# PeterChg/koordinator

Measured on AMD Instinct MI355X. Metric: pod×node Filter+Score evals/sec (LoadAwareScheduling + NodeResourcesFit, matrix mode), higher is better.
Workload: dtype int64

## Files before the change

koordinator_amd/csrc/kg_engine.hip:

```cpp
#include <dlfcn.h>
#include <hip/hip_runtime.h>
#include <rccl/rccl.h>
#include <stdarg.h>
#include <stdio.h>
#include <string.h>

#include <algorithm>
#include <map>
#include <unordered_map>
#include <utility>
#include <string>
#include <type_traits>
#include <vector>

#include "kg_comm.h"
#include "kg_common.h"
#include "kg_host.h"

#define KG_POD_CHUNK 64
#define KG_RESOLVE_THREADS 512
#define KG_RESOLVE_LA_T0 448
#define KG_CLS_ITEM_MAX 512
#define KG_MAX_CHUNK KG_PLACE_CHUNK_MAX
#define KG_MAX_TILES 4096
// ... 1386 lines not shown
    }
    if (live && best && KG_IN2(88, p, a.n_pods, tile, a.tiles_total)) atomicMax(&partials[(int64_t)p * a.tiles_total + tile], best);
}

template <bool COMBINE>
__global__ __launch_bounds__(256) __attribute__((amdgpu_waves_per_eu(KG_NUMA2_WPE))) void k_eval_numa2(kg_consts c, kg_planes pl, HotArgs a,
                                                    const kg_pod_dev *__restrict__ pods,
                                                    const kg_node_row *__restrict__ rows,
                                                    unsigned long long *__restrict__ mask,
                                                    uint16_t *__restrict__ scores, uint8_t *__restrict__ numa_scores,
                                                    uint32_t *__restrict__ partials, const int32_t *__restrict__ perm,
                                                    BatchMasks bm, int32_t *queue, int32_t n_items, int32_t seg) {
    const int tid = threadIdx.x, lane = tid & 63;
    const int wave = __builtin_amdgcn_readfirstlane(tid >> 6);
    __shared__ kg_zone_tab_data ztab[256 / 64];
    __shared__ __attribute__((aligned(16))) uint4 lrow_s[256 / 64][KG_NUMA2_PREFETCH ? 2 : 1][64];
    static_assert(sizeof(kg_node_row) % 16 == 0 && sizeof(kg_node_row) <= 64 * 16, "rows are staged as 16-byte words");
    const int n_pb = (a.n_pods + 63) / 64;
    for (int it = 0;; it++) {
        int64_t tile, base;
        int npw, pb;
        if (queue == nullptr) {
            if (it > 0) break;
            tile = (int64_t)a.tile_begin + blockIdx.x;
            pb = blockIdx.y;
            npw = KG_NUMA2_NODES / (int)gridDim.z;
            base = tile * KG_TILE + wave * KG_NUMA2_NODES + (int64_t)blockIdx.z * npw;
        } else {
            int item = 0;
            if (lane == 0) item = atomicAdd(queue, 1);
            item = __builtin_amdgcn_readfirstlane(item);
            if (item >= n_items) break;
            pb = item % n_pb;
            const int run = item / n_pb;
            tile = (int64_t)a.tile_begin + run / (KG_TILE / seg);
            base = (int64_t)a.tile_begin * KG_TILE + (int64_t)run * seg;
            npw = seg;
        }
        const int slot = pb * 64 + lane;
        const bool live = slot < a.n_pods;
        const int p = live && perm ? perm[slot] : slot;
        const kg_pod_dev pd = pods[live ? p : 0];
        numa2_run<COMBINE>(c, pl, a, pd, p, live, tile, base, npw, rows, mask, scores, numa_scores, partials, bm, ztab[wave],
                  &lrow_s[wave][0][0]);
    }
}

__device__ __forceinline__ unsigned long long decode_partial(uint32_t k, int tile) {
    if (k == 0) return 0ull;
    const uint32_t node = (uint32_t)tile * KG_TILE + (KG_TILE - 1) - (k & (KG_TILE - 1));
    return ((unsigned long long)(k >> KG_TILE_SHIFT) << 32) | (0xFFFFFFFFull - node);
}

__global__ void k_top1(const uint32_t *__restrict__ partials, int32_t tiles, int32_t n_pods,
                       unsigned long long *__restrict__ out) {
    const int wave = (blockIdx.x * blockDim.x + threadIdx.x) >> 6;
    const int lane = threadIdx.x & 63;
    if (wave >= n_pods) return;
    unsigned long long best = 0;
    for (int t = lane; t < tiles; t += 64) {
        unsigned long long k = KG_IN2(89, wave, n_pods, t, tiles) ? decode_partial(partials[(int64_t)wave * tiles + t], t) : 0ull;
        best = best > k ? best : k;
    }
    best = wave_max_u64(best);
    if (lane == 0 && KG_IN(90, wave, n_pods)) out[wave] = best;
}

template <bool NUMA>
__device__ unsigned long long pair_key(const kg_consts &c, const kg_planes &pl, const kg_pod_dev &p, int64_t node,
                                       int64_t n_nodes, int64_t now_ns) {
    if (node < 0 || node >= n_nodes) return 0ull;
    NodeRegs n;
    BatchMasks bm{0xFFu, 0xFFu};
    load_node(c, pl, node, true, bm, now_ns, n);
    uint32_t fit, la, numa = 0;
    if (!eval_pair(c, pl, p, n, node, now_ns, fit, la)) return 0ull;
    if (NUMA && (c.plugins & KG_PLUGIN_NUMA)) {
        const uint64_t ns = kg_numa_eval_any(c, pl.rows[node], p);
        if (!(ns >> 32)) return 0ull;
        numa = (uint32_t)ns;
    }
    return ((unsigned long long)(total_of(c, fit, la, numa) + 1u) << 32) | (0xFFFFFFFFull - (unsigned long long)node);
}

#define KG_NUMA_CHUNK_PODS 16
#define KG_CHUNK_WPE 3
template <bool BZ>
__global__ __launch_bounds__(256) __attribute__((amdgpu_waves_per_eu(KG_CHUNK_WPE))) void k_eval_numa_chunk(kg_consts c, kg_planes pl, HotArgs a,
                                                         const kg_pod_dev *__restrict__ pods, int32_t shard_tiles,
                                                         uint32_t *__restrict__ partials) {
    __shared__ __attribute__((aligned(16))) kg_pod_dev lp;
    __shared__ __attribute__((aligned(16))) uint32_t kbuf[KG_TILE];
    const int tid = threadIdx.x, lane = tid & 63;
    const int n = a.n_pods;
    const int b = blockIdx.x, xcd = b % KG_XCDS, r = b / KG_XCDS;
    const int tile_rel = (r / n) * KG_XCDS + xcd, p = r % n;
    if (tile_rel >= shard_tiles) return;
    constexpr int POD_DW = (int)(sizeof(kg_pod_dev) / 4);
    for (int k = tid; k < POD_DW; k += 256)
        reinterpret_cast<uint32_t *>(&lp)[k] = reinterpret_cast<const uint32_t *>(pods + p)[k];
    __syncthreads();
    const int tile = a.tile_begin + tile_rel;
    const BatchMasks bm{0xFFu, 0xFFu};
#pragma unroll 1
    for (int v = 0; v < KG_TILE / 256; v++) {
        const int local = v * 256 + tid;
        const int64_t node = (int64_t)tile * KG_TILE + local;
        const bool in_range = node < a.node_end;
        NodeRegs nr;
        load_node(c, pl, node, in_range, bm, a.now_ns, nr);
        uint32_t key = 0;
        uint32_t fit, la;
        if (in_range && eval_pair(c, pl, lp, nr, node, a.now_ns, fit, la)) {
// ... 1122 lines not shown
    kg_pod_dev *pods = nullptr;
    void *hot = nullptr;
    int32_t nslot = 2;
    int32_t slot_res[8] = {0, 1, -1, -1, -1, -1, -1, -1};
    int32_t n_pods = 0, pods_cap = 0;
    size_t hot_bytes = 0;
    int32_t *numa_perm = nullptr;
    bool numa_perm_on = false;
    bool eq_on = false;
    int32_t eq_n = 0;
    kg_pod_dev *eq_pods = nullptr;
    void *eq_hot = nullptr;
    bool reps_in = false;
    int32_t *eq_perm = nullptr;
    bool eq_perm_on = false;
    int32_t *eq_of = nullptr;
    void *eq_mem = nullptr;
    size_t eq_mem_bytes = 0;
    void *ncache_mem = nullptr;
    size_t ncache_bytes = 0;
    uint8_t *ncache = nullptr;
    int64_t ncache_stride = 0;
    bool ncache_live = false;
    BatchMasks bm{0, 0};
    uint32_t forms = 0;
    int64_t numa_resident_wgs = 0;
    int64_t numa_resident_wgs_c = 0;
    int32_t *numa_queue = nullptr;
    int32_t numa_chunk_pods = KG_NUMA_CHUNK_PODS;
    bool la_prod = false;
    bool pow2 = true;
    bool cls_ok = false;
    bool cls_dirty = true;
    int64_t cls_width = -1, cls_tiles = -1;
    std::vector<kg_cls_desc> cls_desc;
    std::vector<std::vector<int32_t>> cls_members;
    std::vector<std::vector<int32_t>> cls_ux;
    std::vector<std::vector<int32_t>> cls_reps;
    std::vector<kg_pod_row> pod_rows_h;
    void *cls_mem = nullptr;
    size_t cls_mem_bytes = 0;
    int32_t cls_nwork = 0;
    int32_t cls_nids = 0;
    int32_t cls_kind_work[12][2] = {};
    size_t cls_work_off = 0, cls_rows_off = 0, cls_ids_off = 0;
    int32_t *xslow_list = nullptr;
    int32_t *xslow_count = nullptr;
    double *hot_lax = nullptr;
    bool lax_ok = false;
    int32_t lax_n = 0, lax_x[KG_LAX] = {};
    int32_t *slow_list = nullptr;
    int32_t *slow_count = nullptr;
    bool slow_valid = false;
    void *scratch = nullptr;
    size_t scratch_bytes = 0;
    uint64_t generation = 0;
    bool stale = false;
    std::vector<uint8_t> node_bind_facts;
    int64_t n_numa_policy_nodes = 0, n_node_bind_nodes = 0, n_no_detail_nodes = 0;
    bool batch_bind = false;
    struct CpuTable {
        int32_t max_ref = 1, strategy = KG_STRATEGY_LEAST_ALLOCATED;
        std::vector<kg_cpu_info> cpus;
    };
    std::unordered_map<int32_t, CpuTable> cpu_tab;
    std::vector<uint8_t> pod_may_bind;
    bool profiling = false;
    int64_t cls_target_blocks = 2048, cls_dup_target_blocks = 4096;
    hipStream_t stream2 = nullptr;
    hipEvent_t ev_fork = nullptr, ev_join = nullptr;
    hipEvent_t ev_res[3] = {};
    void *rsv_mem = nullptr;
    kg_reservation *rsv = nullptr;
    std::vector<int32_t> rsv_perm;
    int32_t n_rsv = 0;
    int32_t *rfirst = nullptr, *rnode = nullptr;
    int32_t n_rn = 0;
    unsigned long long *rsv_e = nullptr;
    int64_t *rsv_o = nullptr;
    kg_rsv_ment *rsv_m = nullptr;
    int32_t *rsv_mn = nullptr;
    unsigned long long *rsv_g = nullptr;
    kg_quota *quota = nullptr;
    int32_t n_quota = 0;
    int32_t max_pod_quota = -1;
    uint8_t *gate = nullptr;
    kg_counters ctr{};
    int64_t ev_acc = 0;
    ncclComm_t comm = nullptr;
    kg_shm_comm *shm = nullptr;
    uint32_t *shm_stage = nullptr;
    uint32_t *comm_word = nullptr;
    unsigned long long *cyc_words = nullptr;
    kg_cycle_out *cyc_out = nullptr;
    int32_t comm_rank = 0, comm_world = 0;
    hipStream_t eval_stream = nullptr;
    static constexpr int kEvalEvents = 4;
    hipEvent_t ev_eval[kEvalEvents] = {};
    const void *ev_eval_buf[kEvalEvents] = {};
    int32_t ev_eval_next = 0;
    static constexpr int kRing = 256;
    hipEvent_t ev0[kRing] = {}, ev1[kRing] = {};
    int64_t ev_count = 0;
    std::string err;
};

// ... 428 lines not shown
    e->cls_width = width;
    e->cls_tiles = shard_tiles;
    e->cls_dirty = false;
    return KG_OK;
}

template <bool MOST, bool FIT_ON, bool LA_ON, bool W1, int KIND, int FORM>
void launch_cls_kind(kg_engine *e, dim3 grid, const HotArgs &a_in, const kg_cls_desc *descs, const kg_cls_work *work,
                     const char *rows, const int32_t *ids, uint64_t *mask, uint16_t *scores, uint32_t *partials,
                     hipStream_t stream) {
    constexpr bool LAU = FORM == 1;
    const int32_t first = e->cls_kind_work[3 * KIND + FORM][0], count = e->cls_kind_work[3 * KIND + FORM][1];
    if (count == 0) return;
#ifdef KG_BOUNDS_CHECK
    HotArgs a = a_in;
    a.cls_ndesc = (int32_t)e->cls_desc.size();
    a.cls_nwork = count;
    a.cls_nids = e->cls_nids;
#else
    const HotArgs &a = a_in;
#endif
    if constexpr (LAU && !LA_ON) return;
    else if constexpr (FORM == 2) {
        const dim3 g1((unsigned)((count + KG_XCDS - 1) / KG_XCDS * KG_XCDS));
        if (mask)
            hipLaunchKernelGGL((k_eval3_dup<MOST, FIT_ON, LA_ON, true, W1, KIND>), g1, dim3(KG_TILE / 2), 0, stream,
                               e->consts, e->pl, a, descs, work + first, count, rows, ids, mask, scores, partials);
        else
            hipLaunchKernelGGL((k_eval3_dup<MOST, FIT_ON, LA_ON, false, W1, KIND>), g1, dim3(KG_TILE / 2), 0, stream,
                               e->consts, e->pl, a, descs, work + first, count, rows, ids, mask, scores, partials);
    } else {
        grid.y = (unsigned)count;
        if (mask)
            hipLaunchKernelGGL((k_eval3<MOST, FIT_ON, LA_ON, true, W1, KIND, LAU>), grid, dim3(KG_TILE / 2), 0, stream,
                               e->consts, e->pl, a, descs, work + first, rows, ids, mask, scores, partials);
        else
            hipLaunchKernelGGL((k_eval3<MOST, FIT_ON, LA_ON, false, W1, KIND, LAU>), grid, dim3(KG_TILE / 2), 0, stream,
                               e->consts, e->pl, a, descs, work + first, rows, ids, mask, scores, partials);
    }
}

template <bool MOST, bool FIT_ON, bool LA_ON, bool W1>
void launch_cls4(kg_engine *e, dim3 grid, const HotArgs &a, uint64_t *mask, uint16_t *scores, uint32_t *partials) {
    const char *m = (const char *)e->cls_mem;
    const kg_cls_desc *descs = (const kg_cls_desc *)m;
    const kg_cls_work *work = (const kg_cls_work *)(m + e->cls_work_off);
    const char *rows = m + e->cls_rows_off;
    const int32_t *ids = (const int32_t *)(m + e->cls_ids_off);
    if (!e->stream2) {
        (void)hipStreamCreateWithFlags(&e->stream2, hipStreamNonBlocking);
        (void)hipEventCreateWithFlags(&e->ev_fork, hipEventDisableTiming);
        (void)hipEventCreateWithFlags(&e->ev_join, hipEventDisableTiming);
    }
    (void)hipEventRecord(e->ev_fork, e->stream);
    (void)hipStreamWaitEvent(e->stream2, e->ev_fork, 0);
    hipStream_t s2 = e->stream2;
#define KG_LAUNCH_KIND(K)                                                                                              \
    launch_cls_kind<MOST, FIT_ON, LA_ON, W1, K, 2>(e, grid, a, descs, work, rows, ids, mask, scores, partials, e->stream); \
    launch_cls_kind<MOST, FIT_ON, LA_ON, W1, K, 1>(e, grid, a, descs, work, rows, ids, mask, scores, partials, e->stream); \
    launch_cls_kind<MOST, FIT_ON, LA_ON, W1, K, 0>(e, grid, a, descs, work, rows, ids, mask, scores, partials, s2)
    KG_LAUNCH_KIND(0);
    KG_LAUNCH_KIND(1);
    KG_LAUNCH_KIND(2);
    KG_LAUNCH_KIND(3);
#undef KG_LAUNCH_KIND
    (void)hipEventRecord(e->ev_join, s2);
    (void)hipStreamWaitEvent(e->stream, e->ev_join, 0);
}

template <bool MOST, bool FIT_ON, bool LA_ON>
void launch_cls3(kg_engine *e, dim3 grid, const HotArgs &a, uint64_t *mask, uint16_t *scores, uint32_t *partials) {
    bool unit = e->consts.weight_fit == 1 && e->consts.weight_la == 1;
    if (LA_ON) unit = unit && e->consts.la_w[0] == 1 && e->consts.la_w[1] == 1;
    for (const kg_cls_desc &d : e->cls_desc)
        for (int f = 0; f < 4; f++) unit = unit && d.fit_w[f] <= 1u && d.uni_w[f] <= 1u;
    if (unit) launch_cls4<MOST, FIT_ON, LA_ON, true>(e, grid, a, mask, scores, partials);
    else launch_cls4<MOST, FIT_ON, LA_ON, false>(e, grid, a, mask, scores, partials);
}

void launch_cls(kg_engine *e, dim3 grid, const HotArgs &a, uint64_t *mask, uint16_t *scores, uint32_t *partials) {
    const bool most = e->consts.fit_most != 0;
    const bool fit = (e->consts.plugins & KG_PLUGIN_FIT) != 0, la = (e->consts.plugins & KG_PLUGIN_LOADAWARE) != 0;
    if (!fit) launch_cls3<false, false, true>(e, grid, a, mask, scores, partials);
    else if (most && la) launch_cls3<true, true, true>(e, grid, a, mask, scores, partials);
    else if (most) launch_cls3<true, true, false>(e, grid, a, mask, scores, partials);
    else if (la) launch_cls3<false, true, true>(e, grid, a, mask, scores, partials);
    else launch_cls3<false, true, false>(e, grid, a, mask, scores, partials);
}

kg_status slow_refresh(kg_engine *e) {
    if (e->slow_valid) return KG_OK;
    HIP_TRY(e, hipMemsetAsync(e->slow_count, 0, sizeof(int32_t), e->stream));
    if (e->n_nodes > 0)
        hipLaunchKernelGGL(k_slow_list, dim3((unsigned)((e->n_nodes + 255) / 256)), dim3(256), 0, e->stream, e->pl.dflags,
                           (int64_t)0, e->n_nodes, e->slow_list, e->slow_count);
    HIP_TRY(e, hipGetLastError());
    e->slow_valid = true;
    return KG_OK;
}

kg_status launch_eval_plain(kg_engine *e, int64_t now_ns, int32_t pod_begin, int32_t n, uint64_t *mask, uint16_t *scores,
                            uint32_t *partials, bool use_cls, bool topk, HotArgs a, int64_t shard_tiles, bool prof = true) {
    if (e->consts.la_extra && !topk && e->lax_ok) {
        a.lax_n = e->lax_n;
        for (int k = 0; k < KG_LAX; k++) {
            a.lax_x[k] = k < e->lax_n ? e->lax_x[k] : 0;
            a.lax_w[k] = k < e->lax_n ? (uint32_t)e->consts.la_wx[e->lax_x[k]] : 0u;
        }
        a.lax_est = e->hot_lax + (int64_t)pod_begin * KG_LAX;
        if (prof && e->profiling) HIP_TRY(e, prof_begin(e));
        dim3 grid((unsigned)shard_tiles, (unsigned)((n + a.pods_per_block - 1) / a.pods_per_block));
        const bool prod = e->la_prod;
#define KG_LAX_LAUNCH(S_)                                                                                               \
        do {                                                                                                            \
            const kg_pod_hot_t<S_> *hp = reinterpret_cast<const kg_pod_hot_t<S_> *>(e->hot) + pod_begin;                \
            if (mask && prod)                                                                                          \
                hipLaunchKernelGGL((k_eval2<S_, false, true, true, false, true>), grid, dim3(KG_BLOCK), 0, e->stream,  \
                                   e->consts, e->pl, a, hp, mask, scores, partials);                                   \
            else if (mask)                                                                                             \
                hipLaunchKernelGGL((k_eval2<S_, false, false, true, false, true>), grid, dim3(KG_BLOCK), 0, e->stream, \
                                   e->consts, e->pl, a, hp, mask, scores, partials);                                   \
            else if (prod)                                                                                             \
                hipLaunchKernelGGL((k_eval2<S_, false, true, false, false, true>), grid, dim3(KG_BLOCK), 0, e->stream, \
                                   e->consts, e->pl, a, hp, mask, scores, partials);                                   \
            else                                                                                                       \
                hipLaunchKernelGGL((k_eval2<S_, false, false, false, false, true>), grid, dim3(KG_BLOCK), 0, e->stream,\
                                   e->consts, e->pl, a, hp, mask, scores, partials);                                   \
        } while (0)
        if (e->nslot == 2) KG_LAX_LAUNCH(2);
        else if (e->nslot == 4) KG_LAX_LAUNCH(4);
        else KG_LAX_LAUNCH(8);
#undef KG_LAX_LAUNCH
        HIP_TRY(e, hipGetLastError());
        if (prof && e->profiling) HIP_TRY(e, prof_end(e));
        HIP_TRY(e, hipMemsetAsync(e->xslow_count, 0, sizeof(int32_t), e->stream));
        if (e->n_nodes > 0)
            hipLaunchKernelGGL(k_slow_list, dim3((unsigned)((e->n_nodes + 255) / 256)), dim3(256), 0, e->stream, e->pl.dflags,
                               (int64_t)0, e->n_nodes, e->xslow_list, e->xslow_count, (uint32_t)KGD_XSLOW);
        hipLaunchKernelGGL(k_fix_slow, dim3((unsigned)((n + 255) / 256)), dim3(256), 0, e->stream, e->consts, e->pl,
                           e->pods + pod_begin, n, e->xslow_list, e->xslow_count, e->shard_begin, e->shard_end,
                           a.mask_words, a.score_stride, a.tiles_total, now_ns, (unsigned long long *)mask, scores,
                           partials);
        HIP_TRY(e, hipGetLastError());
        return KG_OK;
    }
    if (e->consts.la_extra && !topk) {
        if (prof && e->profiling) HIP_TRY(e, prof_begin(e));
        const int64_t width = e->shard_end - e->shard_begin;
        dim3 grid((unsigned)((width + 255) / 256), (unsigned)(n < 65535 ? n : 65535));
        hipLaunchKernelGGL(k_eval_exact, grid, dim3(256), 0, e->stream, e->consts, e->pl, e->pods + pod_begin, n,
                           e->shard_begin, e->shard_end, a.mask_words, a.score_stride, a.tiles_total, now_ns,
                           (unsigned long long *)mask, scores, partials);
        HIP_TRY(e, hipGetLastError());
        if (prof && e->profiling) HIP_TRY(e, prof_end(e));
        return KG_OK;
    }
    use_cls = use_cls && e->cls_ok && !e->reps_in && pod_begin == 0 && n == e->n_pods;
    if (use_cls) {
        kg_status st = cls_layout(e, e->shard_end - e->shard_begin, shard_tiles);
        if (st) return st;
    }
    dim3 grid((unsigned)shard_tiles, use_cls ? (unsigned)e->cls_nwork : (unsigned)((n + a.pods_per_block - 1) / a.pods_per_block));
    if (prof && e->profiling) HIP_TRY(e, prof_begin(e));
    if (use_cls) launch_cls(e, grid, a, mask, scores, partials);
    else if (e->nslot == 2) launch_hot<2>(e, grid, a, pod_begin, mask, scores, partials, topk);
    else if (e->nslot == 4) launch_hot<4>(e, grid, a, pod_begin, mask, scores, partials, topk);
    else launch_hot<8>(e, grid, a, pod_begin, mask, scores, partials, topk);
    HIP_TRY(e, hipGetLastError());
    if (prof && e->profiling) HIP_TRY(e, prof_end(e));
    kg_status st = slow_refresh(e);
    if (st) return st;
    if (!topk) {
        hipLaunchKernelGGL(k_fix_slow, dim3((unsigned)((n + 255) / 256)), dim3(256), 0, e->stream, e->consts, e->pl,
                           e->pods + pod_begin, n, e->slow_list, e->slow_count, e->shard_begin, e->shard_end,
                           a.mask_words, a.score_stride, a.tiles_total, now_ns, (unsigned long long *)mask, scores,
                           partials);
        HIP_TRY(e, hipGetLastError());
    }
    return KG_OK;
}

kg_status launch_eval(kg_engine *e, int64_t now_ns, int32_t pod_begin, int32_t n, uint64_t *mask, uint16_t *scores,
                      uint32_t *partials, bool use_cls = false, uint8_t *numa_scores = nullptr, bool topk = false) {
    if (n <= 0) return KG_OK;
    if ((mask == nullptr) != (scores == nullptr)) return set_err(e, KG_ERR_INVALID_ARG, "mask and scores go together");
    const int64_t shard_tiles = (e->shard_end - e->shard_begin + KG_TILE - 1) / KG_TILE;
    if (shard_tiles <= 0) return KG_OK;
    HotArgs a;
    a.n_pods = n;
    a.pods_per_block = pods_per_block_for(n, shard_tiles);
    a.tile_begin = (int32_t)(e->shard_begin / KG_TILE);
    a.tiles_total = (int32_t)tiles_total(e);
    a.node_end = e->shard_end;
    a.col_begin = e->shard_begin;
    a.mask_words = (int32_t)((e->shard_end - e->shard_begin + 63) / 64);
    a.score_stride = (e->shard_end - e->shard_begin + 63) / 64 * 64;
    a.fit_cap = e->consts.fit_most ? 100u : 0xFFFFFFFFu;
    for (int s = 0; s < 8; s++) a.slot_res[s] = s < e->nslot ? e->slot_res[s] : -1;
    a.now_ns = now_ns;
    if ((e->consts.plugins & KG_PLUGIN_NUMA) && topk && n <= e->numa_chunk_pods) {
        if (e->profiling) HIP_TRY(e, prof_begin(e));
        const unsigned blocks = (unsigned)((shard_tiles + KG_XCDS - 1) / KG_XCDS * KG_XCDS * n);
        if (e->ncache_live && !e->consts.numa_bz)
            hipLaunchKernelGGL(k_eval_numa_cached, dim3(blocks), dim3(256), 0, e->stream, e->consts, e->pl, a,
                               e->pods + pod_begin, (int32_t)shard_tiles, partials, e->ncache, e->eq_of + pod_begin,
                               e->ncache_stride, e->eq_n);
        else if (e->consts.numa_bz)
            hipLaunchKernelGGL(k_eval_numa_chunk<true>, dim3(blocks), dim3(256), 0, e->stream, e->consts, e->pl, a,
                               e->pods + pod_begin, (int32_t)shard_tiles, partials);
        else
            hipLaunchKernelGGL(k_eval_numa_chunk<false>, dim3(blocks), dim3(256), 0, e->stream, e->consts, e->pl, a,
                               e->pods + pod_begin, (int32_t)shard_tiles, partials);
        HIP_TRY(e, hipGetLastError());
        if (e->profiling) HIP_TRY(e, prof_end(e));
        return KG_OK;
    }
    if (e->consts.plugins & KG_PLUGIN_NUMA) {
        const bool combine = mask && scores && partials && !topk && !(e->forms & KG_FORM_NUMA_FUSED) &&
                             !(e->reps_in && (e->consts.la_extra || !e->eq_hot));
        if (e->profiling) HIP_TRY(e, prof_begin(e));
        if (combine) {
            kg_status st = launch_eval_plain(e, now_ns, pod_begin, n, mask, scores, partials, use_cls, false, a, shard_tiles,
                                             false);
            if (st) return st;
            HIP_TRY(e, hipMemsetAsync(partials, 0, (size_t)n * (size_t)a.tiles_total * 4, e->stream));
// ... 138 lines not shown
}

extern "C" {

kg_status kg_engine_create(const kg_config *cfg, kg_engine **out) {
    if (!out) return KG_ERR_INVALID_ARG;
    *out = nullptr;
    char msg[256] = {0};
    kg_status st = kg_config_validate(cfg, msg, sizeof(msg));
    if (st != KG_OK) {
        fprintf(stderr, "kg_engine_create: %s\n", msg);
        return st;
    }
    kg_engine *e = new kg_engine();
    e->cfg = *cfg;
    kg_consts_from_config(*cfg, e->consts);
    e->device = cfg->device;
    int ndev = 0;
    if (hipGetDeviceCount(&ndev) != hipSuccess || ndev <= e->device || e->device < 0) {
        fprintf(stderr, "kg_engine_create: no HIP device %d (found %d)\n", e->device, ndev);
        delete e;
        return KG_ERR_HIP;
    }
    if (hipSetDevice(e->device) != hipSuccess || hipStreamCreateWithFlags(&e->stream, hipStreamNonBlocking) != hipSuccess) {
        delete e;
        return KG_ERR_HIP;
    }
    e->own_stream = true;
    *out = e;
    return KG_OK;
}

void kg_engine_destroy(kg_engine *e) {
    if (!e) return;
    (void)hipSetDevice(e->device);
    if (e->stream) (void)hipStreamSynchronize(e->stream);
    if (e->plane_mem) (void)hipFree(e->plane_mem);
    if (e->pods) (void)hipFree(e->pods);
    if (e->hot) (void)hipFree(e->hot);
    if (e->eq_hot) (void)hipFree(e->eq_hot);
    if (e->scratch) (void)hipFree(e->scratch);
    if (e->cls_mem) (void)hipFree(e->cls_mem);
    if (e->rsv_mem) (void)hipFree(e->rsv_mem);
    if (e->quota) (void)hipFree(e->quota);
    if (e->gate) (void)hipFree(e->gate);
    if (e->numa_perm) (void)hipFree(e->numa_perm);
    if (e->numa_queue) (void)hipFree(e->numa_queue);
    if (e->comm) (void)rccl().comm_destroy(e->comm);
    if (e->shm) kg_shm_comm_close(e->shm);
    if (e->shm_stage) (void)hipHostFree(e->shm_stage);
    if (e->comm_word) (void)hipFree(e->comm_word);
    if (e->cyc_words) (void)hipFree(e->cyc_words);
    if (e->cyc_out) (void)hipHostFree(e->cyc_out);
    if (e->hot_lax) (void)hipFree(e->hot_lax);
    if (e->eq_pods) (void)hipFree(e->eq_pods);
    if (e->eq_perm) (void)hipFree(e->eq_perm);
    if (e->eq_of) (void)hipFree(e->eq_of);
    if (e->eq_mem) (void)hipFree(e->eq_mem);
    if (e->ncache_mem) (void)hipFree(e->ncache_mem);
    if (e->own_stream && e->stream) (void)hipStreamDestroy(e->stream);
    if (e->stream2) (void)hipStreamDestroy(e->stream2);
    if (e->ev_fork) (void)hipEventDestroy(e->ev_fork);
    for (int k = 0; k < kg_engine::kEvalEvents; k++)
        if (e->ev_eval[k]) (void)hipEventDestroy(e->ev_eval[k]);
    if (e->ev_join) (void)hipEventDestroy(e->ev_join);
    for (int k = 0; k < 3; k++)
        if (e->ev_res[k]) (void)hipEventDestroy(e->ev_res[k]);
    for (int k = 0; k < kg_engine::kRing; k++) {
        if (e->ev0[k]) (void)hipEventDestroy(e->ev0[k]);
        if (e->ev1[k]) (void)hipEventDestroy(e->ev1[k]);
    }
    delete e;
}

const char *kg_last_error(const kg_engine *e) { return e ? e->err.c_str() : "null engine"; }

kg_status kg_set_stream(kg_engine *e, void *s) {
    kg_status st = check_engine(e);
    if (st) return st;
    HIP_TRY(e, hipStreamSynchronize(e->stream));
    if (e->own_stream) HIP_TRY(e, hipStreamDestroy(e->stream));
    if (s) {
        e->stream = (hipStream_t)s;
        e->own_stream = false;
    } else {
        HIP_TRY(e, hipStreamCreateWithFlags(&e->stream, hipStreamNonBlocking));
        e->own_stream = true;
    }
    return KG_OK;
}

kg_status kg_sync(kg_engine *e) {
    kg_status st = check_engine(e);
    if (st) return st;
    HIP_TRY(e, hipStreamSynchronize(e->stream));
    return KG_OK;
}

kg_status kg_snapshot_reset(kg_engine *e, int32_t n_nodes) {
    kg_status st = check_engine(e, true);
    if (st) return st;
    if (n_nodes < 0) return set_err(e, KG_ERR_INVALID_ARG, "negative node count");
    HIP_TRY(e, hipStreamSynchronize(e->stream));
    if (e->plane_mem) HIP_TRY(e, hipFree(e->plane_mem));
    e->plane_mem = nullptr;
    const int64_t cap = ((int64_t)n_nodes + KG_TILE - 1) / KG_TILE * KG_TILE + (n_nodes == 0 ? KG_TILE : 0);
// ... 352 lines not shown
    const size_t score_b = (size_t)P * (size_t)((width + 63) / 64 * 64) * 2;
    const size_t part_b = (size_t)P * (size_t)T * 4;
    const size_t top_b = (size_t)P * 8;
    auto up = [](size_t b) { return (b + 255) / 256 * 256; };
    const bool dev = out->out_on_device != 0;
    const bool planes = out->mask || out->scores;
    const bool stage_mask = planes && (!dev || !out->mask);
    const bool stage_scores = planes && (!dev || !out->scores);
    const size_t numa_b = (size_t)P * (size_t)((width + 63) / 64 * 64);
    const bool numa_on = (e->consts.plugins & KG_PLUGIN_NUMA) != 0;
    e->ctr.eval_calls++;
    e->ctr.evals += (uint64_t)P * (uint64_t)width;
    e->ctr.out_bytes += (out->mask ? mask_b : 0) + (out->scores ? score_b : 0) + (out->top1 ? top_b : 0) +
                        (out->numa_scores ? numa_b : 0) + (out->rsv_scores ? numa_b : 0);
    const bool stage_numa = out->numa_scores && !dev;
    const bool stage_rsv = out->rsv_scores && !dev;
    size_t need = up(part_b) + up(top_b) + (stage_mask ? up(mask_b) : 0) + (stage_scores ? up(score_b) : 0) +
                  (stage_numa ? up(numa_b) : 0) + (stage_rsv ? up(numa_b) : 0);
    st = ensure_scratch(e, need + 256);
    if (st) return st;
    char *s = (char *)e->scratch;
    uint32_t *part = (uint32_t *)s;
    unsigned long long *top = (unsigned long long *)(s + up(part_b));
    char *q = s + up(part_b) + up(top_b);
    uint64_t *mask = nullptr;
    uint16_t *scores = nullptr;
    if (planes) {
        if (stage_mask) { mask = (uint64_t *)q; q += up(mask_b); }
        else mask = out->mask;
        if (stage_scores) { scores = (uint16_t *)q; q += up(score_b); }
        else scores = (uint16_t *)out->scores;
    }
    uint8_t *numa = nullptr;
    if (out->numa_scores) {
        if (stage_numa) { numa = (uint8_t *)q; q += up(numa_b); }
        else numa = out->numa_scores;
        if (!numa_on && numa_b) HIP_TRY(e, hipMemsetAsync(numa, 0, numa_b, e->stream));
    }
    uint8_t *rsvp = nullptr;
    if (out->rsv_scores) {
        if (stage_rsv) { rsvp = (uint8_t *)q; q += up(numa_b); }
        else rsvp = out->rsv_scores;
        if (numa_b) HIP_TRY(e, hipMemsetAsync(rsvp, 0, numa_b, e->stream));
    }
    const RsvArgs ra = rsv_args(e);
    st = quota_ready(e);
    if (st) return st;
    const bool gated = (ra.quota || ra.rsv) && P > 0;
    if (gated) {
        hipLaunchKernelGGL(k_pod_gate, dim3((unsigned)((P + 255) / 256)), dim3(256), 0, e->stream, ra.quota, ra.quota_parent, e->pods, P,
                           e->gate);
        HIP_TRY(e, hipGetLastError());
    }
    HIP_TRY(e, hipMemsetAsync(part, 0, part_b, e->stream));
    st = launch_eval(e, now_ns, 0, P, mask, scores, part, true, numa_on ? numa : nullptr);
    if (st) return st;
    unsigned long long *tdst = out->top1 ? (dev ? (unsigned long long *)out->top1 : top) : nullptr;
    if (tdst && P > 0) {
        hipLaunchKernelGGL(k_top1, dim3((unsigned)((P + 3) / 4)), dim3(256), 0, e->stream, part, (int32_t)T, P, tdst);
        HIP_TRY(e, hipGetLastError());
    }
    const int32_t mask_words = (int32_t)((width + 63) / 64);
    const int64_t stride = (width + 63) / 64 * 64;
    if (gated) {
        hipLaunchKernelGGL(k_quota_apply, dim3((unsigned)P), dim3(256), 0, e->stream, e->gate + P, P,
                           (unsigned long long *)mask, mask_words, tdst, (uint8_t *)nullptr, stride);
        HIP_TRY(e, hipGetLastError());
    }
    if (ra.rsv) {
        for (int32_t b = 0; b < P; b += KG_RSV_POD_CHUNK) {
            const int32_t n = P - b < KG_RSV_POD_CHUNK ? P - b : KG_RSV_POD_CHUNK;
            st = rsv_eval_chunk(e, now_ns, b, n, mask ? mask + (int64_t)b * mask_words : nullptr,
                                scores ? scores + (int64_t)b * stride : nullptr,
                                numa_on && numa ? numa + (int64_t)b * stride : nullptr, mask_words, stride);
            if (st) return st;
            hipLaunchKernelGGL(k_rsv_reduce, dim3((unsigned)n), dim3(256), 0, e->stream, e->consts, ra, n,
                               tdst ? tdst + b : nullptr, rsvp ? rsvp + (int64_t)b * stride : nullptr, e->shard_begin,
                               e->shard_end, stride);
            HIP_TRY(e, hipGetLastError());
        }
    }
    if (ra.quota && P > 0) {
        hipLaunchKernelGGL(k_quota_apply, dim3((unsigned)P), dim3(256), 0, e->stream, e->gate, P,
                           (unsigned long long *)mask, mask_words, tdst, rsvp, stride);
        HIP_TRY(e, hipGetLastError());
    }
    if (!dev) {
        if (out->top1 && P > 0) HIP_TRY(e, hipMemcpyAsync(out->top1, top, top_b, hipMemcpyDeviceToHost, e->stream));
        if (out->mask && P > 0) HIP_TRY(e, hipMemcpyAsync(out->mask, mask, mask_b, hipMemcpyDeviceToHost, e->stream));
        if (out->scores && P > 0) HIP_TRY(e, hipMemcpyAsync(out->scores, scores, score_b, hipMemcpyDeviceToHost, e->stream));
        if (out->numa_scores && P > 0) HIP_TRY(e, hipMemcpyAsync(out->numa_scores, numa, numa_b, hipMemcpyDeviceToHost, e->stream));
        if (out->rsv_scores && P > 0) HIP_TRY(e, hipMemcpyAsync(out->rsv_scores, rsvp, numa_b, hipMemcpyDeviceToHost, e->stream));
        HIP_TRY(e, hipStreamSynchronize(e->stream));
    }
    return bounds_verdict(e);
}

}

namespace {

kg_status eval_eq(kg_engine *e, int64_t now_ns, const kg_eval_out *out) {
    const int32_t P = e->n_pods, U = e->eq_n;
    const int64_t width = e->shard_end - e->shard_begin;
    const int64_t words = (width + 63) / 64, stride = words * 64;
    const size_t rb[5] = {(size_t)words * 8, (size_t)stride * 2, 8, (size_t)stride, (size_t)stride};
    void *const want[5] = {out->mask, out->scores, out->top1, out->numa_scores, out->rsv_scores};
    const bool dev = out->out_on_device != 0;
    auto up = [](size_t b) { return (b + 255) / 256 * 256; };
    size_t need = 0, off_c[5] = {}, off_s[5] = {};
    for (int k = 0; k < 5; k++)
        if (want[k]) { off_c[k] = need; need += up(rb[k] * (size_t)U); }
// ... 58 lines not shown
    }
    return bounds_verdict(e);
}

kg_status chunk_eval(kg_engine *e, int64_t now_ns, int32_t pod_begin, int32_t n, uint32_t *partial_dev) {
    if (pod_begin < 0 || n < 0 || pod_begin + (int64_t)n > e->n_pods || (n > 0 && !partial_dev))
        return set_err(e, KG_ERR_RANGE, "bad chunk");
    e->ctr.eval_calls++;
    e->ctr.evals += (uint64_t)n * (uint64_t)(e->shard_end - e->shard_begin);
    const bool whole = e->shard_begin == 0 && e->shard_end == e->n_nodes;
    if (((e->consts.plugins & KG_PLUGIN_NUMA) && n > e->numa_chunk_pods) || !whole)
        HIP_TRY(e, hipMemsetAsync(partial_dev, 0, (size_t)n * (size_t)tiles_total(e) * 4 * KG_PARTIAL_SLOTS, e->stream));
    kg_status st = launch_eval(e, now_ns, pod_begin, n, nullptr, nullptr, partial_dev, false, nullptr, true);
    if (st) return st;
    if (rsv_args(e).rsv) {
        if (n > KG_RSV_POD_CHUNK) return set_err(e, KG_ERR_RANGE, "chunk larger than the reservation entry buffer");
        return rsv_eval_chunk(e, now_ns, pod_begin, n, nullptr, nullptr, nullptr, 0, 0, true);
    }
    return KG_OK;
}

kg_status chunk_resolve(kg_engine *e, int64_t now_ns, int32_t pod_begin, int32_t n, const uint32_t *partial_dev,
                        int32_t *out_node_dev, int64_t *out_score_dev, bool defer_last,
                        const int32_t *prev_nodes_dev = nullptr, int32_t n_prev = 0,
                        unsigned long long *pvkeys = nullptr) {
    if (pod_begin < 0 || n < 0 || n > KG_MAX_CHUNK || pod_begin + (int64_t)n > e->n_pods)
        return set_err(e, KG_ERR_RANGE, "bad chunk");
    if (n == 0) return KG_OK;
    kg_status st = quota_ready(e);
    if (st) return st;
    e->ctr.resolved += (uint64_t)n;
    RsvArgs ra = rsv_args(e);
    if (ra.rsv) {
        if (n > KG_RSV_POD_CHUNK) return set_err(e, KG_ERR_RANGE, "chunk larger than the reservation entry buffer");
    }
    st = slow_refresh(e);
    if (st) return st;
    const bool numa = (e->consts.plugins & KG_PLUGIN_NUMA) != 0;
    const bool pv = numa && pvkeys && n_prev > 0 && !ra.rsv && n <= KG_NUMA_CHUNK_PODS && n_prev <= KG_NUMA_CHUNK_PODS;
    if (pv) {
        hipLaunchKernelGGL(k_prev_keys, dim3((unsigned)(n * n_prev)), dim3(64), 0, e->stream, e->consts, e->pl,
                           e->pods + pod_begin, n, prev_nodes_dev, n_prev, e->n_nodes, now_ns, pvkeys);
        HIP_TRY(e, hipGetLastError());
    }
    auto *kres = ra.rsv ? (numa ? k_resolve<true, true> : k_resolve<true, false>)
                        : (numa ? k_resolve<false, true> : k_resolve<false, false>);
    hipLaunchKernelGGL(kres, dim3(1), dim3(KG_RESOLVE_THREADS), 0, e->stream,
                       e->consts, e->pl, e->pods, pod_begin, n,
                       partial_dev, (int32_t)tiles_total(e), e->n_nodes, now_ns, out_node_dev, out_score_dev, ra,
                       numa && n > e->numa_chunk_pods ? 1 : KG_PARTIAL_SLOTS, e->slow_list, e->slow_count,
                       numa ? 0 : 1,
                       defer_last ? 1 : 0, prev_nodes_dev, n_prev, pv ? pvkeys : nullptr);
    HIP_TRY(e, hipGetLastError());
    e->generation++;
    return KG_OK;
}

constexpr size_t kHostRowOff = 0, kHostNodeOff = (sizeof(kg_node_row) + 255) / 256 * 256;
constexpr size_t kHostReserveHead = kHostNodeOff + 256;
static_assert(kHostNodeOff >= kHostRowOff + sizeof(kg_node_row) && kHostNodeOff + 4 <= kHostReserveHead,
              "the row and its node index fit the head");
kg_status host_reserve(kg_engine *e, int32_t pod, int32_t node, bool *failed) {
    *failed = false;
    kg_node_row row;
    HIP_TRY(e, hipMemcpyAsync(&row, e->pl.rows + node, sizeof(row), hipMemcpyDeviceToHost, e->stream));
    HIP_TRY(e, hipStreamSynchronize(e->stream));
    kg_pod_dev pd;
    kg_pod_dev_from_row(e->cfg, e->pod_rows_h[(size_t)pod], pd);
    int required, take;
    const bool bind = (e->consts.plugins & KG_PLUGIN_NUMA) && kg_numa_binds(row, pd, required, take);
    std::vector<uint8_t> taken;
    kg_engine::CpuTable *tab = nullptr;
    if (bind) {
        auto it = e->cpu_tab.find(node);
        if (it == e->cpu_tab.end())
            return set_err(e, KG_ERR_STATE, "node %d: cpuset Reserve needs the node's CPUs (kg_cpus_set)", node);
        tab = &it->second;
        const int32_t nc = (int32_t)tab->cpus.size();
        taken.assign((size_t)nc, 0);
        if (kg_cpuset_allocate(e->consts, row, pd, required, take, tab->cpus.data(), nc, tab->max_ref, tab->strategy,
                               taken.data()) != 0) {
            *failed = true;
            return KG_OK;
        }
    }
    hipLaunchKernelGGL(k_commit_one, dim3(1), dim3(1), 0, e->stream, e->consts, e->pl, e->pods, pod, node, rsv_args(e));
    HIP_TRY(e, hipGetLastError());
    if (bind) {
        const int32_t nc = (int32_t)tab->cpus.size();
        kg_cpuset_apply(pd, tab->cpus.data(), nc, taken.data());
        HIP_TRY(e, hipMemcpyAsync(&row, e->pl.rows + node, sizeof(row), hipMemcpyDeviceToHost, e->stream));
        HIP_TRY(e, hipStreamSynchronize(e->stream));
        kg_cpuset_row_fields(row, tab->cpus.data(), nc, tab->max_ref);
        kg_status st = ensure_scratch(e, kHostReserveHead);
        if (st) return st;
        char *sc = (char *)e->scratch;
        HIP_TRY(e, h2d(e, sc + kHostRowOff, &row, sizeof(row), e->stream));
        HIP_TRY(e, h2d(e, sc + kHostNodeOff, &node, 4, e->stream));
        hipLaunchKernelGGL(k_upsert, dim3(1), dim3(256), 0, e->stream, e->consts, e->pl, (const kg_node_row *)(sc + kHostRowOff),
                           (const int32_t *)(sc + kHostNodeOff), 1);
        HIP_TRY(e, hipGetLastError());
    }
    HIP_TRY(e, hipStreamSynchronize(e->stream));
    e->slow_valid = false;
    e->generation++;
    return KG_OK;
// ... 874 lines not shown
```

Before: 2408 billion.

## Skip redundant partials memset, slow-fix kernel, and cross-stream fork when unneeded

Several small launch eliminations in the matrix eval path. A pinned host mirror of the slow-node count lets the host skip launching k_fix_slow when no slow nodes exist. The partials memset is skipped when the class path covers the whole batch, and k_top1 scans only this shard's tile range. The stream2 fork/join events are recorded only when that stream actually gets work. The risk is correctness: the memset skip assumes the class kernels write every partial, and the host mirror can be stale if it is not invalidated in all the right places.

```diff
diff --git a/koordinator_amd/csrc/kg_engine.hip b/koordinator_amd/csrc/kg_engine.hip
--- a/koordinator_amd/csrc/kg_engine.hip
+++ b/koordinator_amd/csrc/kg_engine.hip
@@ -1462,13 +1462,13 @@
     return ((unsigned long long)(k >> KG_TILE_SHIFT) << 32) | (0xFFFFFFFFull - node);
 }
 
-__global__ void k_top1(const uint32_t *__restrict__ partials, int32_t tiles, int32_t n_pods,
-                       unsigned long long *__restrict__ out) {
+__global__ void k_top1(const uint32_t *__restrict__ partials, int32_t tiles, int32_t tile_begin, int32_t tile_end,
+                       int32_t n_pods, unsigned long long *__restrict__ out) {
     const int wave = (blockIdx.x * blockDim.x + threadIdx.x) >> 6;
     const int lane = threadIdx.x & 63;
     if (wave >= n_pods) return;
     unsigned long long best = 0;
-    for (int t = lane; t < tiles; t += 64) {
+    for (int t = tile_begin + lane; t < tile_end; t += 64) {
         unsigned long long k = KG_IN2(89, wave, n_pods, t, tiles) ? decode_partial(partials[(int64_t)wave * tiles + t], t) : 0ull;
         best = best > k ? best : k;
     }
@@ -2697,6 +2697,9 @@
     int32_t *slow_list = nullptr;
     int32_t *slow_count = nullptr;
     bool slow_valid = false;
+    int32_t *slow_count_h = nullptr;
+    hipEvent_t ev_slow = nullptr;
+    bool slow_mirror = false;
     void *scratch = nullptr;
     size_t scratch_bytes = 0;
     uint64_t generation = 0;
@@ -3231,8 +3234,12 @@
         (void)hipEventCreateWithFlags(&e->ev_fork, hipEventDisableTiming);
         (void)hipEventCreateWithFlags(&e->ev_join, hipEventDisableTiming);
     }
-    (void)hipEventRecord(e->ev_fork, e->stream);
-    (void)hipStreamWaitEvent(e->stream2, e->ev_fork, 0);
+    bool mixed = false;
+    for (int k = 0; k < 4; k++) mixed = mixed || e->cls_kind_work[3 * k + 0][1] != 0;
+    if (mixed) {
+        (void)hipEventRecord(e->ev_fork, e->stream);
+        (void)hipStreamWaitEvent(e->stream2, e->ev_fork, 0);
+    }
     hipStream_t s2 = e->stream2;
 #define KG_LAUNCH_KIND(K)                                                                                              \
     launch_cls_kind<MOST, FIT_ON, LA_ON, W1, K, 2>(e, grid, a, descs, work, rows, ids, mask, scores, partials, e->stream); \
@@ -3243,8 +3250,10 @@
     KG_LAUNCH_KIND(2);
     KG_LAUNCH_KIND(3);
 #undef KG_LAUNCH_KIND
-    (void)hipEventRecord(e->ev_join, s2);
-    (void)hipStreamWaitEvent(e->stream, e->ev_join, 0);
+    if (mixed) {
+        (void)hipEventRecord(e->ev_join, s2);
+        (void)hipStreamWaitEvent(e->stream, e->ev_join, 0);
+    }
 }
 
 template <bool MOST, bool FIT_ON, bool LA_ON>
@@ -3274,8 +3283,29 @@
         hipLaunchKernelGGL(k_slow_list, dim3((unsigned)((e->n_nodes + 255) / 256)), dim3(256), 0, e->stream, e->pl.dflags,
                            (int64_t)0, e->n_nodes, e->slow_list, e->slow_count);
     HIP_TRY(e, hipGetLastError());
+    if (!e->slow_count_h) {
+        HIP_TRY(e, hipHostMalloc((void **)&e->slow_count_h, sizeof(int32_t), hipHostMallocDefault));
+        HIP_TRY(e, hipEventCreateWithFlags(&e->ev_slow, hipEventDisableTiming));
+    }
+    HIP_TRY(e, hipMemcpyAsync(e->slow_count_h, e->slow_count, sizeof(int32_t), hipMemcpyDeviceToHost, e->stream));
+    HIP_TRY(e, hipEventRecord(e->ev_slow, e->stream));
+    e->slow_mirror = true;
     e->slow_valid = true;
     return KG_OK;
+}
+
+bool slow_known_empty(kg_engine *e) {
+    if (!e->slow_valid || !e->slow_mirror) return false;
+    if (hipEventQuery(e->ev_slow) != hipSuccess) {
+        (void)hipGetLastError();
+        return false;
+    }
+    return *(const volatile int32_t *)e->slow_count_h == 0;
+}
+
+bool cls_whole_batch(const kg_engine *e, bool use_cls, bool topk, int32_t pod_begin, int32_t n) {
+    if (e->consts.la_extra && !topk) return false;
+    return use_cls && e->cls_ok && !e->reps_in && pod_begin == 0 && n == e->n_pods;
 }
 
 kg_status launch_eval_plain(kg_engine *e, int64_t now_ns, int32_t pod_begin, int32_t n, uint64_t *mask, uint16_t *scores,
@@ -3334,7 +3364,7 @@
         if (prof && e->profiling) HIP_TRY(e, prof_end(e));
         return KG_OK;
     }
-    use_cls = use_cls && e->cls_ok && !e->reps_in && pod_begin == 0 && n == e->n_pods;
+    use_cls = cls_whole_batch(e, use_cls, topk, pod_begin, n);
     if (use_cls) {
         kg_status st = cls_layout(e, e->shard_end - e->shard_begin, shard_tiles);
         if (st) return st;
@@ -3349,7 +3379,7 @@
     if (prof && e->profiling) HIP_TRY(e, prof_end(e));
     kg_status st = slow_refresh(e);
     if (st) return st;
-    if (!topk) {
+    if (!topk && !slow_known_empty(e)) {
         hipLaunchKernelGGL(k_fix_slow, dim3((unsigned)((n + 255) / 256)), dim3(256), 0, e->stream, e->consts, e->pl,
                            e->pods + pod_begin, n, e->slow_list, e->slow_count, e->shard_begin, e->shard_end,
                            a.mask_words, a.score_stride, a.tiles_total, now_ns, (unsigned long long *)mask, scores,
@@ -3594,6 +3624,8 @@
     if (e->comm_word) (void)hipFree(e->comm_word);
     if (e->cyc_words) (void)hipFree(e->cyc_words);
     if (e->cyc_out) (void)hipHostFree(e->cyc_out);
+    if (e->slow_count_h) (void)hipHostFree(e->slow_count_h);
+    if (e->ev_slow) (void)hipEventDestroy(e->ev_slow);
     if (e->hot_lax) (void)hipFree(e->hot_lax);
     if (e->eq_pods) (void)hipFree(e->eq_pods);
     if (e->eq_perm) (void)hipFree(e->eq_perm);
@@ -4052,12 +4084,14 @@
                            e->gate);
         HIP_TRY(e, hipGetLastError());
     }
-    HIP_TRY(e, hipMemsetAsync(part, 0, part_b, e->stream));
+    if (numa_on || !cls_whole_batch(e, true, false, 0, P)) HIP_TRY(e, hipMemsetAsync(part, 0, part_b, e->stream));
     st = launch_eval(e, now_ns, 0, P, mask, scores, part, true, numa_on ? numa : nullptr);
     if (st) return st;
     unsigned long long *tdst = out->top1 ? (dev ? (unsigned long long *)out->top1 : top) : nullptr;
     if (tdst && P > 0) {
-        hipLaunchKernelGGL(k_top1, dim3((unsigned)((P + 3) / 4)), dim3(256), 0, e->stream, part, (int32_t)T, P, tdst);
+        const int32_t t0 = (int32_t)(e->shard_begin / KG_TILE);
+        const int32_t t1 = t0 + (int32_t)((width + KG_TILE - 1) / KG_TILE);
+        hipLaunchKernelGGL(k_top1, dim3((unsigned)((P + 3) / 4)), dim3(256), 0, e->stream, part, (int32_t)T, t0, t1, P, tdst);
         HIP_TRY(e, hipGetLastError());
     }
     const int32_t mask_words = (int32_t)((width + 63) / 64);
@@ -4222,6 +4256,7 @@
                        numa ? 0 : 1,
                        defer_last ? 1 : 0, prev_nodes_dev, n_prev, pv ? pvkeys : nullptr);
     HIP_TRY(e, hipGetLastError());
+    e->slow_mirror = false;
     e->generation++;
     return KG_OK;
 }
```

Result: faster. 2552 billion (median of 6 runs) (+6.0%).
